# wenxuanliu/multimodal-vae

Hardware: AMD Instinct MI355X
Metric: ELBO-steps/sec (whole node), MultiMNIST b=256 per GPU (higher is better)
Workload: dtype bf16; 1 GPU; multimnist_50x50_conv_mmvae_gru_text_3pass_elbo_step; batch_per_gpu=256, global_batch=256, n_latents=100, parallelism=dp1, hip_graph=False, optimizer=adam, mfma=bf16 in / fp32 acc; fp32 master weights, BN stats, PoE/KL/BCE/NLL, Adam

## Files before the change

multimodal-vae_amd/csrc/elementwise.hip:

```cpp
#include "elementwise.h"
#include "bn_dev.h"
#include <math.h>

namespace {

constexpr int TPB = 256;

__device__ __forceinline__ float exp_unfused(float x) {
    const float c = 0x1.715476p+0f, cc = 0x1.4ae0bep-26f;
    float ph = x * c;
    asm volatile("" : "+v"(ph));
    float pl = fmaf(x, c, -ph);
    pl = fmaf(x, cc, pl);
    const float e = rintf(ph);
    float r = ldexpf(__builtin_amdgcn_exp2f((ph - e) + pl), (int)e);
    r = x < -0x1.9d1dap+6f ? 0.f : r;
    r = x > 0x1.62e43p+6f ? INFINITY : r;
    return r;
}
inline int nblocks(long long n, int per = TPB, int cap = 4096) {
    long long b = (n + per - 1) / per;
    if (b < 1) b = 1;
    if (b > cap) b = cap;
    return (int)b;
// ... 666 lines not shown
        a.z_bf[(size_t)b * a.ldz + a.D + c] = (bf16)(c == 0 ? 1.f : 0.f);
    }
    __shared__ double part[TPB / 64];
    kl = wave_sum_f64(kl);
    if ((threadIdx.x & 63) == 0) part[threadIdx.x >> 6] = kl;
    __syncthreads();
    if (threadIdx.x == 0) {
        double s = 0.0;
        for (int w = 0; w < TPB / 64; ++w) s += part[w];
        reinterpret_cast<double*>(a.scratch)[blockIdx.x] = s;
    }
}
__global__ void latent1_fwd_finish_kernel(const double* parts, float* kl_sum) {
    if (threadIdx.x != 0 || blockIdx.x != 0) return;
    double s = 0.0;
    for (int p = 0; p < LATENT1_KL_PARTS; ++p) s += parts[p];
    *kl_sum += (float)s;
}
__global__ __launch_bounds__(TPB) void latent1_bwd_kernel(const Latent1BwdArgs a) {
    const Latent1Args& f = a.f;
    const int D2 = 2 * f.D;
    const int tx = threadIdx.x & 63, ty = threadIdx.x >> 6;
    const int d = blockIdx.x * 64 + tx;
    __shared__ double red[2][4][64];
    double s_mu = 0.0, s_lv = 0.0;
    const int b_end = min(f.B, (int)(blockIdx.y + 1) * LATENT1_BWD_ROWS);
    for (int b = blockIdx.y * LATENT1_BWD_ROWS + ty; b < b_end; b += 4) {
        if (d < f.D) {
            const int e = b * f.D + d;
            double dz = a.dz ? (double)a.dz[e] : 0.0;
            if (a.dz2) dz += (double)a.dz2[e];
            const double mu = f.mu[e], lv = f.logvar[e], kc = a.kl_coef;
            const double gmu = dz + kc * mu;
            double glv = -0.5 * kc * (1.0 - exp(lv));
            if (f.training) glv += dz * (double)f.eps[e] * 0.5 * exp(0.5 * lv);
            a.d_enc_out[(size_t)b * a.ld + d] = (bf16)(float)gmu;
            a.d_enc_out[(size_t)b * a.ld + f.D + d] = (bf16)(float)glv;
            s_mu += gmu; s_lv += glv;
        }
        if (blockIdx.x == 0)
            for (int c = D2 + tx; c < a.ld; c += 64) a.d_enc_out[(size_t)b * a.ld + c] = (bf16)0.f;
    }
    if (!a.d_bias) return;
    red[0][ty][tx] = s_mu; red[1][ty][tx] = s_lv;
    __syncthreads();
    if (ty == 0 && d < f.D) {
        double* row = reinterpret_cast<double*>(f.scratch) + (size_t)blockIdx.y * D2;
        row[d] = red[0][0][tx] + red[0][1][tx] + red[0][2][tx] + red[0][3][tx];
        row[f.D + d] = red[1][0][tx] + red[1][1][tx] + red[1][2][tx] + red[1][3][tx];
    }
}
__global__ __launch_bounds__(TPB) void latent1_bwd_finish_kernel(const double* parts, int nrows, int D2, float* d_bias, const float* loss_slots,
                                                                 float* loss_out) {
    const int c = threadIdx.x;
    if (loss_slots && c < 16) {
        float t = 0.f;
        for (int q = 0; q < MMVAE_LOSS_SLOTS; ++q) t += loss_slots[q * 16 + c];
        loss_out[c] = t;
    }
    if (!d_bias || c >= D2) return;
    double s = 0.0;
    for (int r = 0; r < nrows; ++r) s += parts[(size_t)r * D2 + c];
    d_bias[c] += (float)s;
}
__global__ __launch_bounds__(TPB) void latent1_bwd_f32_kernel(const Latent1BwdF32Args a) {
    const long long n = (long long)a.B * a.ld;
    for (long long i = (long long)blockIdx.x * TPB + threadIdx.x; i < n; i += (long long)gridDim.x * TPB) {
        const int b = (int)(i / a.ld), c = (int)(i - (long long)b * a.ld);
        float v = 0.f;
        if (c < 2 * a.D) {
            const bool is_mu = c < a.D;
            const int e = b * a.D + (is_mu ? c : c - a.D);
            const double dz = a.dz ? (double)a.dz[e] : 0.0;
            const double mu = a.mu[e], lv = a.logvar[e], kc = a.kl_coef;
            const double gmu = dz + kc * mu;
            double glv = -0.5 * kc * (1.0 - exp(lv));
            if (a.training) glv += dz * (double)a.eps[e] * 0.5 * exp(0.5 * lv);
            v = is_mu ? (float)gmu : (float)glv;
        }
        a.d_enc_out[i] = v;
    }
}

__global__ __launch_bounds__(TPB) void adam_kernel(const AdamArgs a, unsigned* done) {
    const long long t = *a.step + 1;
    const bool skip = done[1] != 0u || (__float_as_uint(a.g[0]) & 0x7fffffffu) == MMVAE_VOID_MARK;
    const float bc1 = 1.0f - powf(a.b1, (float)t);
    const float bc2 = 1.0f - powf(a.b2, (float)t);
    const float step_size = a.lr / bc1;
    const float inv_sqrt_bc2 = rsqrtf(bc2);
    long long vbase[5];
    vbase[0] = 0;
#pragma unroll
    for (int r = 0; r < 4; ++r) vbase[r + 1] = vbase[r] + (r < a.nr ? (a.rlen[r] + 3) / 4 : 0);
    for (long long i = (long long)blockIdx.x * TPB + threadIdx.x; i < vbase[4] && !skip; i += (long long)gridDim.x * TPB) {
        int r = 0;
#pragma unroll
        for (int q = 1; q < 4; ++q) r += (q < a.nr && i >= vbase[q]) ? 1 : 0;
        const long long e = a.roff[r] + (i - vbase[r]) * 4, r_end = a.roff[r] + a.rlen[r];
        if (e + 4 <= r_end) {
            f32x4 g = *reinterpret_cast<const f32x4*>(a.g + e);
            if (a.gmap) {
                const int4 mi = *reinterpret_cast<const int4*>(a.gmap + e);
                const int mm[4] = {mi.x, mi.y, mi.z, mi.w};
#pragma unroll
                for (int j = 0; j < 4; ++j)
                    if (mm[j] >= 0) g[j] += a.gpk[mm[j]];
                    else if (mm[j] < -1) g[j] += a.gpk_vec[-mm[j] - 2];
                *reinterpret_cast<f32x4*>(a.g_out + e) = g;
            }
            f32x4 m = *reinterpret_cast<const f32x4*>(a.m + e);
            f32x4 v = *reinterpret_cast<const f32x4*>(a.v + e);
            f32x4 p = *reinterpret_cast<const f32x4*>(a.p + e);
#pragma unroll
            for (int j = 0; j < 4; ++j) {
                float gj = g[j] * a.grad_scale;
                m[j] = a.b1 * m[j] + (1.f - a.b1) * gj;
                v[j] = a.b2 * v[j] + (1.f - a.b2) * gj * gj;
                p[j] -= step_size * m[j] / (sqrtf(v[j]) * inv_sqrt_bc2 + a.eps);
            }
            *reinterpret_cast<f32x4*>(a.m + e) = m;
            *reinterpret_cast<f32x4*>(a.v + e) = v;
            *reinterpret_cast<f32x4*>(a.p + e) = p;
        } else {
            for (long long q = e; q < r_end; ++q) {
                float gq = a.g[q];
                if (a.gmap) {
                    const int mq = a.gmap[q];
                    if (mq >= 0) gq += a.gpk[mq]; else if (mq < -1) gq += a.gpk_vec[-mq - 2];
                    a.g_out[q] = gq;
                }
                float gj = gq * a.grad_scale;
                float m = a.b1 * a.m[q] + (1.f - a.b1) * gj;
                float v = a.b2 * a.v[q] + (1.f - a.b2) * gj * gj;
                a.m[q] = m; a.v[q] = v;
                a.p[q] -= step_size * m / (sqrtf(v) * inv_sqrt_bc2 + a.eps);
            }
        }
    }
    __syncthreads();
    if (threadIdx.x == 0) {
        unsigned ticket = atomicAdd(done, 1u);
        if (ticket == gridDim.x - 1) {
            done[0] = 0u;
            done[1] = 0u;
            if (!skip && !a.no_advance) *a.step = t;
            __threadfence();
        }
    }
}

__global__ __launch_bounds__(TPB) void embed_gather_stats_kernel(const float* table, int C, const long long* idx, int rows, int idx_rows,
                                                                 int rows_per_group, bf16* x, int ld, float2* colstats) {
    const int r0 = blockIdx.x * 64;
    for (int c = threadIdx.x & 63; c < ld; c += 64) {
        float s1 = 0.f, s2 = 0.f;
        int g_cur = -1;
        for (int rr = threadIdx.x >> 6; rr < 64; rr += TPB / 64) {
            const int r = r0 + rr;
            if (r >= rows) break;
            const int g = r / rows_per_group;
            if (g != g_cur && g_cur >= 0 && c < C && colstats) {
                atomicAdd(&colstats[(g_cur * MMVAE_STAT_SLOTS + blockIdx.x % MMVAE_STAT_SLOTS) * C + c].x, s1);
                atomicAdd(&colstats[(g_cur * MMVAE_STAT_SLOTS + blockIdx.x % MMVAE_STAT_SLOTS) * C + c].y, s2);
                s1 = s2 = 0.f;
            }
            g_cur = g;
            float v = 0.f;
            if (c < C) v = table[idx[r % idx_rows] * C + c];
            const bf16 b = (bf16)v;
            x[(size_t)r * ld + c] = b;
            const float vb = (float)b;
            s1 += vb; s2 += vb * vb;
        }
        if (g_cur >= 0 && c < C && colstats) {
            atomicAdd(&colstats[(g_cur * MMVAE_STAT_SLOTS + blockIdx.x % MMVAE_STAT_SLOTS) * C + c].x, s1);
            atomicAdd(&colstats[(g_cur * MMVAE_STAT_SLOTS + blockIdx.x % MMVAE_STAT_SLOTS) * C + c].y, s2);
        }
    }
}
__global__ __launch_bounds__(TPB) void embed_scatter_add_kernel(const bf16* d, int ld, int C, const long long* idx, int rows, float* g_table) {
    const int i = blockIdx.x * TPB + threadIdx.x;
    if (i >= rows * C) return;
    const int r = i / C, c = i - r * C;
    atomicAdd(g_table + idx[r] * C + c, (float)d[(size_t)r * ld + c]);
}
__global__ __launch_bounds__(TPB) void logsoftmax_nll_kernel(const LogSoftmaxNllArgs a) {
    const int r = blockIdx.x * TPB + threadIdx.x;
    float nll = 0.f;
    int g = 0;
    if (r < a.rows) {
        g = r / a.rows_per_group;
        const float* l = a.logits + (size_t)r * a.classes;
        float mx = -INFINITY;
        for (int c = 0; c < a.classes; ++c) mx = fmaxf(mx, l[c]);
        float se = 0.f;
        for (int c = 0; c < a.classes; ++c) se += exp_unfused(l[c] - mx);
        const float lg = logf(se);
        const int tg = a.target ? (int)a.target[r % a.target_rows] : -1;
        for (int c = 0; c < a.classes; ++c) {
            const float lp = (l[c] - mx) - lg;
            a.words[(size_t)r * a.classes + c] = lp;
            if (c == tg) nll = -lp;
            if (a.dlogits) a.dlogits[(size_t)r * a.ld_d + c] = (bf16)(a.coef[g & 3] * (exp_unfused(lp) - (c == tg ? 1.f : 0.f)));
            if (a.dlogits_f32) a.dlogits_f32[(size_t)r * a.classes + c] = a.coef[g & 3] * (exp_unfused(lp) - (c == tg ? 1.f : 0.f));
        }
        if (a.dlogits)
            for (int c = a.classes; c < a.ld_d; ++c) a.dlogits[(size_t)r * a.ld_d + c] = (bf16)0.f;
    }
    if (a.nll_sum && a.target) {
        if (a.rows_per_group % 64 == 0) {
            float s = wave_sum(nll);
            if ((threadIdx.x & 63) == 0 && r < a.rows) atomicAdd(a.nll_sum + (blockIdx.x % MMVAE_LOSS_SLOTS) * 16 + g, s);
        } else if (r < a.rows) {
            atomicAdd(a.nll_sum + (r % MMVAE_LOSS_SLOTS) * 16 + g, nll);
        }
    }
}
__global__ __launch_bounds__(TPB) void cast_bf16_kernel(const float* x, long long n, bf16* out) {
    const long long i = ((long long)blockIdx.x * TPB + threadIdx.x) * 4;
    if (i + 4 <= n) {
        const f32x4 v = *reinterpret_cast<const f32x4*>(x + i);
        bf16x4 o;
        for (int j = 0; j < 4; ++j) o[j] = (bf16)v[j];
        *reinterpret_cast<bf16x4*>(out + i) = o;
    } else {
        for (long long q = i; q < n; ++q) out[q] = (bf16)x[q];
    }
}
__global__ __launch_bounds__(TPB) void mse_fwd_kernel(const float* a, const float* b, long long n, float* out) {
    float acc = 0.f;
    for (long long i = (long long)blockIdx.x * TPB + threadIdx.x; i < n; i += (long long)gridDim.x * TPB) {
        const float d = a[i] - b[i];
        acc += d * d;
// ... 206 lines not shown
    MMVAE_REQUIRE(out != nullptr && n >= 0, "normal: null output or n=%lld < 0", n);
    if (n == 0) return MMVAE_OK;
    hipLaunchKernelGGL(normal_kernel, dim3(nblocks((n + 3) / 4, TPB, 512)), dim3(TPB), 0, s, out, n, seed, step, stream_id);
    return mmvae_check_launch("normal");
}
int launch_keep_mask(uint8_t* out, long long n, float p, unsigned long long seed, const long long* step, unsigned stream_id, hipStream_t s) {
    MMVAE_REQUIRE(out != nullptr && n >= 0, "keep_mask: null output or n=%lld < 0", n);
    MMVAE_REQUIRE(p >= 0.0f && p <= 1.0f, "keep_mask: p=%g is no probability in [0, 1]", (double)p);
    if (n == 0) return MMVAE_OK;
    hipLaunchKernelGGL(keep_mask_kernel, dim3(nblocks((n + 3) / 4, TPB, 512)), dim3(TPB), 0, s, out, n, p, seed, step, stream_id);
    return mmvae_check_launch("keep_mask");
}
int launch_latent3_fwd(const Latent3Args& a, hipStream_t s) {
    MMVAE_REQUIRE(a.B >= 1 && a.D >= 1 && a.ldz >= a.D && a.ldz % 8 == 0 && (long long)a.B * a.ldz <= 0x3FFFFFFF,
                  "latent3: B=%d D=%d ldz=%d", a.B, a.D, a.ldz);
    MMVAE_REQUIRE(a.img_out && a.txt_out && a.mu && a.logvar && a.z_f32 && a.z_bf && a.kl_sum && (!a.training || a.eps), "latent3: null argument");
    MMVAE_LAUNCH(latent3_fwd_kernel, dim3(nblocks((long long)a.B * a.ldz, TPB, 256)), dim3(TPB), 0, s, a);
    return mmvae_check_launch("latent3_fwd");
}
int launch_latent3_bwd(const Latent3BwdArgs& a, hipStream_t s) {
    MMVAE_REQUIRE((a.loss_slots == nullptr) == (a.loss_out == nullptr), "latent3_bwd: loss_slots / loss_out go together");
    MMVAE_REQUIRE(a.f.B >= 1 && a.f.D >= 1 && (long long)a.f.B * a.f.D <= 0x3FFFFFFF && ceil_div(a.f.B, L3B_ROWS) <= 65535,
                  "latent3_bwd: B=%d D=%d out of range", a.f.B, a.f.D);
    MMVAE_REQUIRE(a.f.img_out && a.f.txt_out && a.f.mu && a.f.logvar && (!a.f.training || a.f.eps), "latent3_bwd: null argument");
    MMVAE_REQUIRE(a.d_img_out_f32 || a.d_img_out_bf, "latent3_bwd: no image gradient output (d_img_out_f32 or d_img_out_bf)");
    MMVAE_REQUIRE(a.ld_img_out_bf == 0 || (a.ld_img_out_bf >= 2 * a.f.D && a.ld_img_out_bf % 8 == 0),
                  "latent3_bwd: ld_img_out_bf=%d is no multiple of 8 >= 2D", a.ld_img_out_bf);
    MMVAE_LAUNCH(latent3_bwd_kernel, dim3(ceil_div(a.f.D, 64), ceil_div(a.f.B, L3B_ROWS)), dim3(TPB), 0, s, a);
    return mmvae_check_launch("latent3_bwd");
}
size_t launch_latent1_scratch_floats(int B, int D) {
    const size_t fwd = 2 * (size_t)LATENT1_KL_PARTS, bwd = 2 * (size_t)ceil_div(B, LATENT1_BWD_ROWS) * 2 * D;
    return bwd > fwd ? bwd : fwd;
}
static int latent1_check(const Latent1Args& a, const char* who) {
    MMVAE_REQUIRE(a.B >= 1 && a.D >= 1 && a.D <= 128 && (long long)a.B * a.D <= 0x3FFFFFFF, "%s: B=%d D=%d out of range (D <= 128)", who, a.B, a.D);
    MMVAE_REQUIRE(a.mu && a.logvar && a.scratch && (!a.training || a.eps), "%s: null argument", who);
    MMVAE_REQUIRE(((uintptr_t)a.scratch & 7) == 0, "%s: scratch must be 8-byte aligned", who);
    return MMVAE_OK;
}
int launch_latent1_fwd(const Latent1Args& a, hipStream_t s) {
    MMVAE_TRY(latent1_check(a, "latent1_fwd"));
    MMVAE_REQUIRE(a.enc_out && a.z_f32 && a.z_bf && a.kl_sum, "latent1_fwd: null argument");
    MMVAE_REQUIRE(a.ldz >= a.D, "latent1_fwd: ldz=%d < D=%d", a.ldz, a.D);
    hipLaunchKernelGGL(latent1_fwd_kernel, dim3(LATENT1_KL_PARTS), dim3(TPB), 0, s, a);
    MMVAE_TRY(mmvae_check_launch("latent1_fwd"));
    MMVAE_LAUNCH(latent1_fwd_finish_kernel, dim3(1), dim3(64), 0, s, (const double*)a.scratch, a.kl_sum);
    return mmvae_check_launch("latent1_fwd_finish");
}
int launch_latent1_bwd(const Latent1BwdArgs& a, hipStream_t s) {
    MMVAE_TRY(latent1_check(a.f, "latent1_bwd"));
    MMVAE_REQUIRE(a.d_enc_out && a.ld >= 2 * a.f.D, "latent1_bwd: d_enc_out missing or ld=%d < 2D", a.ld);
    MMVAE_REQUIRE((a.loss_slots == nullptr) == (a.loss_out == nullptr), "latent1_bwd: loss_slots / loss_out go together");
    const int nrows = ceil_div(a.f.B, LATENT1_BWD_ROWS);
    hipLaunchKernelGGL(latent1_bwd_kernel, dim3(ceil_div(a.f.D, 64), nrows), dim3(TPB), 0, s, a);
    MMVAE_TRY(mmvae_check_launch("latent1_bwd"));
    if (!a.d_bias && !a.loss_slots) return MMVAE_OK;
    MMVAE_LAUNCH(latent1_bwd_finish_kernel, dim3(1), dim3(TPB), 0, s, (const double*)a.f.scratch, nrows, 2 * a.f.D, a.d_bias, a.loss_slots, a.loss_out);
    return mmvae_check_launch("latent1_bwd_finish");
}
int launch_latent1_bwd_f32(const Latent1BwdF32Args& a, hipStream_t s) {
    MMVAE_REQUIRE(a.B >= 1 && a.D >= 1 && a.D <= 128 && (long long)a.B * a.D <= 0x3FFFFFFF, "latent1_bwd_f32: B=%d D=%d out of range (D <= 128)", a.B, a.D);
    MMVAE_REQUIRE(a.mu && a.logvar && a.d_enc_out && (!a.training || a.eps), "latent1_bwd_f32: null argument");
    MMVAE_REQUIRE(a.ld >= 2 * a.D && (long long)a.B * a.ld <= 0x3FFFFFFF, "latent1_bwd_f32: ld=%d out of range (>= 2D)", a.ld);
    const int nb = ceil_div(a.B * a.ld, TPB);
    hipLaunchKernelGGL(latent1_bwd_f32_kernel, dim3(nb < 1024 ? nb : 1024), dim3(TPB), 0, s, a);
    return mmvae_check_launch("latent1_bwd_f32");
}
int launch_adam(const AdamArgs& a_in, hipStream_t s) {
    AdamArgs a = a_in;
    MMVAE_REQUIRE(a.step != nullptr, "adam: step counter is null");
    MMVAE_REQUIRE(a.p && a.g && a.m && a.v, "adam: null parameter, gradient or moment buffer");
    MMVAE_REQUIRE(a.n >= 1, "adam: n=%lld elements (the kernel reads g[0])", a.n);
    MMVAE_REQUIRE(a.gmap == nullptr || (a.gpk && a.gpk_vec && a.g_out), "adam: gradient map without packed gradient buffers");
    MMVAE_REQUIRE(a.nr >= 0 && a.nr <= 4, "adam: at most 4 element ranges");
    if (a.nr == 0) { a.nr = 1; a.roff[0] = 0; a.rlen[0] = a.n; }
    long long vecs = 0;
    for (int r = 0; r < a.nr; ++r) {
        MMVAE_REQUIRE(a.roff[r] >= 0 && a.rlen[r] >= 0 && a.roff[r] % 4 == 0 && a.roff[r] + a.rlen[r] <= a.n &&
                      (a.rlen[r] % 4 == 0 || a.roff[r] + a.rlen[r] == a.n), "adam: range %d = (%lld, %lld) of %lld elements", r, a.roff[r], a.rlen[r], a.n);
        vecs += (a.rlen[r] + 3) / 4;
    }
    unsigned* done = reinterpret_cast<unsigned*>(a.step + 1);
    hipLaunchKernelGGL(adam_kernel, dim3(nblocks(vecs > 0 ? vecs : 1, TPB, mmvae_knob(K_adam_blocks))), dim3(TPB), 0, s, a, done);
    return mmvae_check_launch("adam");
}
static __global__ __launch_bounds__(256) void gather_rows_kernel(const char* __restrict__ src, const long long* __restrict__ idx,
                                                                 long long row_bytes, int parts, char* __restrict__ dst) {
    const long long row = blockIdx.x / parts;
    const int part = blockIdx.x % parts;
    const long long vecs = row_bytes / 16, per = (vecs + parts - 1) / parts;
    const long long v0 = part * per, v1 = v0 + per < vecs ? v0 + per : vecs;
    const u32x4* s = reinterpret_cast<const u32x4*>(src + idx[row] * row_bytes);
    u32x4* d = reinterpret_cast<u32x4*>(dst + row * row_bytes);
    for (long long v = v0 + threadIdx.x; v < v1; v += 256) d[v] = s[v];
}
static __global__ __launch_bounds__(256) void gather_rows4_kernel(const char* __restrict__ src, const long long* __restrict__ idx,
                                                                  long long row_bytes, char* __restrict__ dst) {
    const long long row = blockIdx.x;
    const unsigned* s = reinterpret_cast<const unsigned*>(src + idx[row] * row_bytes);
    unsigned* d = reinterpret_cast<unsigned*>(dst + row * row_bytes);
    for (long long v = threadIdx.x; v < row_bytes / 4; v += 256) d[v] = s[v];
}
static __global__ __launch_bounds__(256) void gather_rows_u8_f32_kernel(const unsigned char* __restrict__ src, const long long* __restrict__ idx,
                                                                       long long row_elems, float denom, float* __restrict__ dst) {
    const long long row = blockIdx.x;
    const unsigned* s = reinterpret_cast<const unsigned*>(src + idx[row] * row_elems);
    f32x4* d = reinterpret_cast<f32x4*>(dst + row * row_elems);
    for (long long v = threadIdx.x; v < row_elems / 4; v += 256) {
        const unsigned w = s[v];
        d[v] = f32x4{(float)(w & 255u) / denom, (float)((w >> 8) & 255u) / denom, (float)((w >> 16) & 255u) / denom, (float)(w >> 24) / denom};
    }
}
int launch_gather_rows_u8_f32(const unsigned char* src, const long long* idx, long long rows, long long row_elems, float denom, float* dst, hipStream_t s) {
    MMVAE_REQUIRE(src && idx && dst && rows >= 1 && rows < (1ll << 31) && row_elems >= 4 && row_elems % 4 == 0 && ((uintptr_t)src & 3) == 0 &&
                  ((uintptr_t)dst & 15) == 0, "gather_rows_u8_f32: rows of a multiple of 4 elements, aligned buffers");
    hipLaunchKernelGGL(gather_rows_u8_f32_kernel, dim3((unsigned)rows), dim3(256), 0, s, src, idx, row_elems, denom, dst);
    return mmvae_check_launch("gather_rows_u8_f32");
}
int launch_gather_rows(const void* src, const long long* idx, long long rows, long long row_bytes, void* dst, hipStream_t s) {
    if (src && idx && dst && rows >= 1 && row_bytes >= 4 && row_bytes % 16 != 0) {
        MMVAE_REQUIRE(row_bytes % 4 == 0 && ((uintptr_t)src & 3) == 0 && ((uintptr_t)dst & 3) == 0 && rows < (1ll << 31), "gather_rows: rows of a multiple of 4 bytes, 4-byte aligned buffers");
        hipLaunchKernelGGL(gather_rows4_kernel, dim3((unsigned)rows), dim3(256), 0, s, (const char*)src, idx, row_bytes, (char*)dst);
        return mmvae_check_launch("gather_rows");
    }
    MMVAE_REQUIRE(src && idx && dst && rows >= 1 && row_bytes >= 16 && row_bytes % 16 == 0, "gather_rows: rows of a multiple of 16 bytes");
    MMVAE_REQUIRE(((uintptr_t)src & 15) == 0 && ((uintptr_t)dst & 15) == 0, "gather_rows: 16-byte aligned buffers");
    int parts = (int)((row_bytes + 32767) / 32768);
    if (parts < 1) parts = 1;
    MMVAE_REQUIRE(rows * parts < (1ll << 31), "gather_rows: too many rows");
    hipLaunchKernelGGL(gather_rows_kernel, dim3((unsigned)(rows * parts)), dim3(256), 0, s, (const char*)src, idx, row_bytes, parts, (char*)dst);
    return mmvae_check_launch("gather_rows");
}
static __global__ void step_losses_kernel(StepLossArgs a) {
    const int k = threadIdx.x;
    if (k < 3) a.out[k] = a.w_bce[k] * a.sums[k] + a.w_nll[k] * a.sums[4 + k] + a.w_kl[k] * a.sums[8 + k];
}
int launch_step_losses(const StepLossArgs& a, hipStream_t s) {
    MMVAE_REQUIRE(a.sums && a.out, "step_losses: null buffer");
    hipLaunchKernelGGL(step_losses_kernel, dim3(1), dim3(64), 0, s, a);
    return mmvae_check_launch("step_losses");
}
int launch_fill_zero(void* p, size_t bytes, hipStream_t s) {
    if (hipMemsetAsync(p, 0, bytes, s) != hipSuccess) {
        mmvae_set_error("hipMemsetAsync failed");
        return MMVAE_EHIP;
    }
    return MMVAE_OK;
}

int launch_bce_fwd(const float* p, const float* t, long long n, float* out, hipStream_t s) {
    hipLaunchKernelGGL(bce_fwd_kernel, dim3(nblocks(n, TPB * 4, 1024)), dim3(TPB), 0, s, p, t, n, out);
    return mmvae_check_launch("bce_fwd");
}
int launch_bce_bwd(const float* p, const float* t, long long n, float coef, const float* gs, float* dp, hipStream_t s) {
    hipLaunchKernelGGL(bce_bwd_kernel, dim3((unsigned)((n + TPB - 1) / TPB)), dim3(TPB), 0, s, p, t, n, coef, gs, dp);
    return mmvae_check_launch("bce_bwd");
}
int launch_nll_fwd(const float* lp, const long long* tg, int rows, int classes, float* out, hipStream_t s) {
    hipLaunchKernelGGL(nll_fwd_kernel, dim3(nblocks(rows, TPB, 64)), dim3(TPB), 0, s, lp, tg, rows, classes, out);
    return mmvae_check_launch("nll_fwd");
}
int launch_nll_bwd(const long long* tg, int rows, int classes, float coef, const float* gs, float* dlp, hipStream_t s) {
    hipLaunchKernelGGL(nll_bwd_kernel, dim3(ceil_div(rows * classes, TPB)), dim3(TPB), 0, s, tg, rows, classes, coef, gs, dlp);
    return mmvae_check_launch("nll_bwd");
}

// ... 85 lines not shown
```

multimodal-vae_amd/csrc/knobs.h:

```cpp
#pragma once
#include <atomic>

#define MMVAE_KNOBS(KNOB) \
    KNOB(convres, 1, AB, "image-resident conv kernels (convres.hip); 0: every layer on gemm_gather, except launches with a staging transform, which exist only there") \
    KNOB(convres_celeba, 1, AB, "convres.hip on the 64x64 image tower's layers (CelebA, COCO); 0: those layers on gemm_gather") \
    KNOB(convres_alt, 0, AB, "convres.hip tile configurations: 1 hallucinate.6 with 4 images per workgroup, 3 no direct-B kernels, 4 no split bottleneck kernels, 5 no 16-image hallucinate.0") \
    KNOB(convres_dbg, 0, MEASURE, "convres kernels leave phases out (bit mask, tools/convres_check.py)") \
    KNOB(convres_ts_lo, 0, ADDR, "convres kernels: time stamps of workgroup 0's phases, low half of the pointer") \
    KNOB(convres_ts_hi, 0, ADDR, "high half") \
    KNOB(mm_fuse_bn, 1, AB, "MultiMNIST step: BatchNorm passes folded into the staging of the image-resident conv kernels; 0: the unfused bn_act + gather-GEMM chain") \
    KNOB(ca_fuse_bn, 1, AB, "the same for the 64x64 image tower (CelebA, COCO)") \
    KNOB(mm_stage_out, 1, AB, "the staging conv kernels leave the activated operand / BatchNorm-backward dr behind for the weight gradient; 0: materialised on the side stream in front of it") \
    KNOB(mm_conv1_mfma, 1, AB, "MultiMNIST features.0 forward and weight gradient on conv1.hip; 0: gemm_gather") \
    KNOB(dec_last_mfma, 1, AB, "MultiMNIST decoder tail (hallucinate.9 + BCE + its gradients) on dec_last.hip; 0: separate launches") \
    KNOB(dec_last_ca, 1, AB, "the 64x64 tower's decoder tail on dec_last.hip; 0: separate launches") \
    KNOB(dec_last_ca_dbg, 0, MEASURE, "64x64 decoder tail leaves work out: bit 0 logits, 1 patches, 2 input gradient, 3 weight gradient, 4 P") \
    KNOB(wgrad_ring, 1, AB, "ring-staged weight-gradient kernels (wgrad_ring.hip); 0: the streamed gemm_gather form") \
    KNOB(wr_pair, 0, AB, "1: the two-classes-per-workgroup geometries of wgrad_ring.hip (tried and lost, DESIGN)") \
    KNOB(wr_wgs, -1, TUNE, "workgroups of a ring launch in quarters of the CU count; -1: 4 from 4e9 MACs, else 3") \
    KNOB(wr_wgs_big, 0, TUNE, "the same for a geometry that names its own (G::WGQ); 0: the geometry's") \
    KNOB(wr_bias, 6, TUNE, "fixed cost of a batch for a ring workgroup, in column tiles, when image groups are dealt to classes") \
    KNOB(wr_run, 0, TUNE, "consecutive jobs dealt to one XCD residue by the ring launch's workgroup order; 0: one per job class and channel slice") \
    KNOB(wr_xcd, 1, AB, "0: ring jobs in sorted order, not dealt to the XCDs") \
    KNOB(wr_atomic_kb, 256, TUNE, "a ring launch adds into the packed gradient by fp32 atomics up to this many KB of dW; above: partial copies + reduce") \
    KNOB(wr_dbg, 0, MEASURE, "ring kernels leave phases out (bit mask, tools/wgrad_check.py)") \
    KNOB(wr_ts_lo, 0, ADDR, "ring kernels: time stamps of workgroup 0's phases, low half of the pointer") \
    KNOB(wr_ts_hi, 0, ADDR, "high half") \
    KNOB(wgrad_atomic, 0, AB, "1: streamed weight gradients add into the packed gradient by fp32 atomics, no slab / reduce") \
    KNOB(batch_reduce, 1, AB, "one reduce launch per flushed side stream; 0: one behind every weight gradient") \
    KNOB(mm_wgrad_inline, 0, AB, "1: MultiMNIST image weight gradients on the main stream (no fork, no join); 2: and their partial copies summed by one launch in front of the optimizer") \
    KNOB(one_wgrad_stream, 0, AB, "1: one weight-gradient side stream instead of two") \
    KNOB(side_lanes, 3, AB, "bit 0: lane-1 side work goes to the second-modality stream; bit 1: lane 2 to the spare weight-gradient stream") \
    KNOB(mm_cls_lane, 1, AB, "side-stream lane of the classifier's grouped weight gradients") \
    KNOB(mm_conv3_lane, 0, AB, "side-stream lane of features.5's weight gradient") \
    KNOB(mm_conv4_lane, 0, AB, "side-stream lane of features.8's weight gradient") \
    KNOB(mm_forks, 0, AB, "1: one fork for the whole encoder / decoder backward instead of one per flush point") \
    KNOB(one_join, -1, AB, "end of step: 1 the side streams meet on one of them and the main stream waits once, 0 it waits for each; -1: once when there are two weight-gradient streams") \
    KNOB(ev_flags, 2, AB, "flags of the step's events: 2 no system-scope fence, 0 HIP's default fence (read when an event is created)") \
    KNOB(no_stop_events, 0, AB, "1: forks are event records on the main stream, not the producer kernel's completion signal") \
    KNOB(adam_blocks, 512, TUNE, "workgroup cap of the Adam kernel") \
    KNOB(begin_blocks, 2048, TUNE, "zero / random-number workgroup cap of the step prologue") \
    KNOB(mm_dz_event, 1, AB, "the main chain joins the text decoder backward on that kernel's own event; 0: on everything enqueued on its stream") \
    KNOB(mm_stage_begin, 1, AB, "staged prologue: the main stream refreshes only what the image encoder's forward reads, the rest on the second-modality stream; 0: one launch") \
    KNOB(mm_early_adam, 1, AB, "the decoders' Adam update runs beside the encoders' backward when the caller passes early_adam; 0: never") \
    KNOB(mm_image_waist, -1, AB, "image-only MultiMNIST step: 1 / 0 the one-expert waist kernels on / off where compiled; -1: the size's default (1 at n_latents = 20, 0 at 100)") \
    KNOB(mnist_strip, -1, AB, "image-only MNIST step: 1 / 0 the column-strip Linear + BatchNorm kernels on / off up to 512 rows; -1: the default, 1") \
    KNOB(text_fwd2, 1, AB, "MultiMNIST text decoder forward: the weights-resident text_decoder_fwd2_kernel at the reference's sizes; 0: the streamed form at every size") \
    KNOB(txt_ts_lo, 0, ADDR, "text decoder forward: time stamps of workgroup 0's phases, low half of the pointer") \
    KNOB(txt_ts_hi, 0, ADDR, "high half") \
    KNOB(pack_runs, 1, AB, "every weight pack: the lanes of a wave walk the source's contiguous direction (pack_geo.h); 0: the row-major assignment it replaced, reference of tests/test_gpu_pack_runs.py") \
    KNOB(pack_stage_grid, 1, AB, "a staged prologue launch holds only its own descriptors' workgroups and the zero / random workgroups it needs; 0: the whole table and begin_blocks workgroups in every launch") \
    KNOB(gemm_small_prefetch, 2, AB, "gemm_small_kernel with 2 .. 4 64-deep chunks of both operands in flight per wave; 0: gemm_small_kernel_v0, reference of tests/test_gpu_gemm_small_forms.py") \
    KNOB(dbg_skip_wgrad, 0, MEASURE, "the step without weight gradients: 1 all, 2 ring-staged, 3 streamed, 4 grouped") \
    KNOB(dbg_skip_text, 0, MEASURE, "1: the step without its text kernels") \
    KNOB(dbg_skip_edges, 0, MEASURE, "the step without event edges: 1 all, 2 forks (main -> side), 3 joins") \
    KNOB(dbg_begin_skip, 0, MEASURE, "prologue without: bit 0 the pack, 1 the random draws, 2 the workspace zeroing") \
    KNOB(dbg_begin_skip_zero, 0, MEASURE, "prologue without zeroing: bit 0 the packed gradient, 1 the gradients") \
    KNOB(dbg_text_rows_div, 0, MEASURE, "n > 0: the text decoder on 1/n of its rows") \
    KNOB(coco_cluster, 8, AB, "ranks per 16-row block of the caption decoder's persistent launches: 8, 4, or 0 / 1 one workgroup per block") \
    KNOB(coco_enc_streamed, 0, AB, "1: the caption encoder's weight-streaming kernels instead of the weight-resident ones") \
    KNOB(coco_no_comb, 0, AB, "1: the cluster-of-8 decoder's three-exchange kernels instead of the composed two-exchange form") \
    KNOB(coco_no_comb_bwd, 0, AB, "1: the composed form off in the decoder's backward only") \
    KNOB(coco_no_mse_fuse, 0, AB, "1: the caption MSE not fused into the composed decoder forward") \
    KNOB(coco_module_bf16, 0, AB, "caption module entry points: 0 the fp32 kernels; 1 the step's bf16 persistent kernels on the module's B rows; 2 their forward without saving, backward refuses") \
    KNOB(celeba_layer_mask, 0, AB, "mmvae_celeba_bench_layer: 1 the dropout keep flags take part in the fc layers") \
    KNOB(coco_layer_mask, 0, AB, "mmvae_coco_bench_layer: 1 the dropout keep flags in m1 / m2 take part in the fc layers")

enum MmvaeKnob {
#define KNOB(name, dflt, kind, doc) K_##name,
    MMVAE_KNOBS(KNOB)
#undef KNOB
    K_COUNT
};

extern std::atomic<int> g_mmvae_knobs[K_COUNT];
static inline int mmvae_knob(MmvaeKnob k) { return g_mmvae_knobs[k].load(std::memory_order_relaxed); }
static inline unsigned long long* mmvae_knob_ptr(MmvaeKnob lo, MmvaeKnob hi) {
    return reinterpret_cast<unsigned long long*>(((unsigned long long)(unsigned)mmvae_knob(hi) << 32) | (unsigned)mmvae_knob(lo));
}
```

multimodal-vae_amd/csrc/multimnist.hip:

```cpp
#include "multimnist.h"
#include <memory>
#include "mlp_tail.h"
#include "plan_base.h"
#include "thin.h"
#include "text_plan.h"
#include <cstring>

namespace {
constexpr int IMG = 50, NPIX = 2500;
}

struct MMPlan : PlanBase {
    int ldz, kx, kz;
    int lde;
    ConvL conv[4], convT[4];
    LinL fc[3], up;
    BnL bn[6];
    int H = TXT_H;
    const char *te_name = "text_encoder", *td_name = "text_decoder";
    TextGruIdx te_f, te_r, td0, td1;
    const float* step_image = nullptr;
    hipEvent_t ev_dz = nullptr;
    hipEvent_t ev_txtgrads = nullptr;
    int te_h2p, te_h2pT, g_te_h2p, td_z2h, td_z2hT, g_td_z2h, td_h2o, td_h2oT, g_td_h2o;
// ... 700 lines not shown
TextDecArgs td_args(MMPlan& P, const float* z, int groups, bool save) { return text_dec_args(P, z, groups, save); }
int txt_dec_bwd(MMPlan& P, const TextDecArgs& f, const float* dwords, float* dz, hipStream_t s) {
    const int R = f.R;
    const TextDecBwdArgs a = text_dec_bwd_args(P, f, dwords, dz);
    P.ev_dz = nullptr;
    const bool own_ev = P.in_step && s == P.st_text && mmvae_knob(K_mm_dz_event) != 0;
    if (own_ev) {
        P.ev_dz = next_ev(P);
        if (!P.capturing && !mmvae_knob(K_no_stop_events)) mmvae_arm_stop_event(P.ev_dz);
    }
    MMVAE_TRY(launch_text_decoder_bwd(a, s));
    if (own_ev && (mmvae_take_stop_event() != nullptr || P.capturing || mmvae_knob(K_no_stop_events)) && hipEventRecord(P.ev_dz, s) != hipSuccess) {
        mmvae_set_error("text decoder event failed: %s", hipGetErrorString(hipGetLastError()));
        return MMVAE_EHIP;
    }
    MMVAE_TRY(text_dec_wgrads(P, R, s));
    P.ev_txtgrads = nullptr;
    if (own_ev) {
        P.ev_txtgrads = next_ev(P);
        if (hipEventRecord(P.ev_txtgrads, s) != hipSuccess) {
            mmvae_set_error("text decoder event failed: %s", hipGetErrorString(hipGetLastError()));
            return MMVAE_EHIP;
        }
    }
    return MMVAE_OK;
}

}

MMPlan* mm_create(int D, int B) {
    if (D < 1 || D > 127 || B < 1) { mmvae_set_error("mm_create: need 1 <= n_latents <= 127 and batch >= 1"); return nullptr; }
    MMPlan* P = new MMPlan();
    P->D = D; P->B = B;
    P->single_wgrad_stream = true;
    build_plan(*P);
    plan_size_workspaces(*P, carve);
    return P;
}
void mm_destroy(MMPlan* P) { delete P; }
int mm_early_ranges(const MMPlan* P, long long* ranges, int cap) {
    int n = 0;
    for (const ParamInfo& pi : P->params) {
        if (pi.name.rfind("image_decoder.", 0) != 0 && pi.name.rfind("text_decoder.", 0) != 0) continue;
        if (n > 0 && ranges[2 * (n - 1)] + ranges[2 * (n - 1) + 1] == pi.offset) { ranges[2 * (n - 1) + 1] += pi.numel; continue; }
        if (n == cap) return 0;
        ranges[2 * n] = pi.offset; ranges[2 * n + 1] = pi.numel; ++n;
    }
    for (int r = 0; r < n; ++r)
        if (ranges[2 * r] % 4 != 0 || ranges[2 * r + 1] % 4 != 0) return 0;
    return n;
}
PlanBase* mm_base(MMPlan* P) { return P; }

static int use_ws(MMPlan* P, void* ws, size_t bytes, bool module = true) { return plan_use_ws(P, ws, bytes, module, carve); }

static int mm_step_body(MMPlan* Pp, const mmvae_mm_step_io& io, int training, int do_backward, hipStream_t s);
int mm_step_fwd_bwd(MMPlan* Pp, const mmvae_mm_step_io& io, int training, int do_backward, hipStream_t s) {
    if (const mmvae_early_adam* e = io.early_adam) {
        MMVAE_REQUIRE(e->m && e->v && e->state && e->gmap && e->ran, "mmvae_mm_step: early_adam with a null field");
        *e->ran = 0;
    }
    return plan_step(Pp, io, training, do_backward, s, mm_step_body);
}
static int mm_step_body(MMPlan* Pp, const mmvae_mm_step_io& io, int training, int do_backward, hipStream_t s) {
    MMVAE_TRY(use_ws(Pp, io.ws, io.ws_bytes, false));
    MMPlan& P = *Pp;
    MMPlan::W& w = P.w;
    const int B = P.B, D = P.D, B3 = 3 * B;
    MMVAE_REQUIRE(io.image && io.text && io.sums, "step: image/text/sums must be given");
    const float* eps = io.eps;
    const uint8_t *m1 = io.enc_mask1, *m2 = io.enc_mask2, *gk = io.gru_keep;
    const bool serial0 = mmvae_serial();
    const bool staged = mmvae_knob(K_mm_stage_begin) != 0 && !serial0;
    StepBeginArgs sb{}, sb2{};
    sb.zero_ptr[0] = w.zero_begin; sb.zero_bytes[0] = w.zero_bytes;
    StepBeginArgs& sz = staged ? sb2 : sb;
    if (do_backward) {
        sz.zero_ptr[1] = P.buf.gpk; sz.zero_bytes[1] = (size_t)P.gk.mat_elems * sizeof(float);
        sz.zero_ptr[2] = P.buf.grads; sz.zero_bytes[2] = (size_t)(P.nparams / 4) * 16;
        const int skipz = mmvae_knob(K_dbg_begin_skip_zero);
        if (skipz & 1) sz.zero_ptr[1] = nullptr;
        if (skipz & 2) sz.zero_ptr[2] = nullptr;
    }
    sb.p = DROP_P; sb.seed = io.seed; sb.step = io.step_counter;
    if (training && !eps) { sb.eps = w.eps; sb.n_eps = (long long)B3 * D; eps = w.eps; }
    if (training && io.enc_dropout && !m1) { sb.mask[0] = w.m1; sb.n_mask[0] = (long long)2 * B * 400; m1 = w.m1; }
    if (training && io.enc_dropout && !m2) { sb.mask[1] = w.m2; sb.n_mask[1] = (long long)2 * B * 200; m2 = w.m2; }
    if (training && io.gru_dropout && !gk) { sb.mask[2] = w.gkeep; sb.n_mask[2] = (long long)4 * B3 * P.H; gk = w.gkeep; }
    const int skipb = mmvae_knob(K_dbg_begin_skip);
    if (skipb & 2) { sb.eps = nullptr; sb.mask[0] = sb.mask[1] = sb.mask[2] = nullptr; }
    if (skipb & 4) sb.zero_ptr[0] = nullptr;
    const bool pack_now = io.pack_first && !(skipb & 1);
    if (pack_now) {
        MMVAE_TRY(step_begin_with_pack(sb, P.buf.desc_dev, P.pk.d.data(), (int)P.pk.d.size(), P.buf.params, P.buf.packed, P.buf.packed_vec,
                                       staged ? 1u << 0 : 0u));
    }
    MMVAE_TRY(ensure_streams(P));
    P.in_step = true;
    {
        hipStreamCaptureStatus cs = hipStreamCaptureStatusNone;
        P.capturing = hipStreamIsCapturing(s, &cs) == hipSuccess && cs == hipStreamCaptureStatusActive;
    }
    arm_fork(P);
    MMVAE_TRY(launch_step_begin(sb, s));
    MMVAE_TRY(commit_fork(P, s));
    if (do_backward && P.nparams % 4 != 0)
        MMVAE_TRY(launch_fill_zero(P.buf.grads + (P.nparams / 4) * 4, (size_t)(P.nparams % 4) * sizeof(float), s));
    const int enc_drop = training && io.enc_dropout;
    const int sk[3] = {io.pass_skip[0] != 0, io.pass_skip[1] != 0, io.pass_skip[2] != 0};
    P.dec_skip_mask = (unsigned)(sk[0] | (sk[1] << 1) | (sk[2] << 2));
    const int enc_updates = 2 - sk[0] - sk[1];
    const bool serial = mmvae_serial();
    hipStream_t T = serial ? s : P.st_text;
    if (T != s) MMVAE_TRY(fork_to(P, T));
    if (staged && pack_now) {
        StepBeginArgs st1{};
        MMVAE_TRY(step_begin_with_pack(st1, P.buf.desc_dev, P.pk.d.data(), (int)P.pk.d.size(), P.buf.params, P.buf.packed, P.buf.packed_vec, 1u << 1));
        MMVAE_TRY(launch_step_begin(st1, T));
    }
    {
        TextEncArgs a = te_args(P, io.text, w.txtout, do_backward);
        MMVAE_TRY(launch_text_encoder_fwd(a, T));
    }
    if (staged && (pack_now || sb2.zero_ptr[1] || sb2.zero_ptr[2])) {
        if (pack_now)
            MMVAE_TRY(step_begin_with_pack(sb2, P.buf.desc_dev, P.pk.d.data(), (int)P.pk.d.size(), P.buf.params, P.buf.packed, P.buf.packed_vec, 1u << 2));
        MMVAE_TRY(launch_step_begin(sb2, T));
    }
    P.step_image = io.image;
    const bool fuse = mmvae_knob(K_mm_fuse_bn) != 0 && mmvae_knob(K_convres) != 0 && B % 8 == 0;
    MMVAE_TRY(enc_fwd(P, io.image, 2, m1, m2, enc_drop, training, enc_updates, w.encout, s, fuse));
    MMVAE_TRY(edge(P, T, s));
    Latent3Args la{};
    la.B = B; la.D = D; la.img_out = w.encout; la.txt_out = w.txtout; la.eps = eps;
    la.mu = io.mu ? io.mu : w.mu; la.logvar = io.logvar ? io.logvar : w.logvar;
    la.z_f32 = w.z_f32; la.z_bf = w.z_bf; la.ldz = P.ldz; la.kl_sum = w.sums + 8; la.training = training;
    arm_fork(P);
    MMVAE_TRY(launch_latent3_fwd(la, s));
    MMVAE_TRY(commit_fork(P, s));
    if (T != s) MMVAE_TRY(fork_to(P, T));
    TextDecArgs td = td_args(P, w.z_f32, 3, do_backward);
    td.keep = (training && io.gru_dropout) ? gk : nullptr; td.keep_scale = 1.f / (1.f - DROP_P);
    td.force_tokens = io.force_tokens;
    if (io.recon_text) td.words = io.recon_text;
    if (io.tokens) td.tokens_out = io.tokens;
    td.target = io.text; td.nll_sum = w.sums + 4; td.dwords = do_backward ? w.dwords : nullptr;
    for (int k = 0; k < 3; ++k) td.nll_coef[k] = sk[k] ? 0.f : io.lambda_yx[k] / (float)(B * TXT_T);
    if (const int half = mmvae_knob(K_dbg_text_rows_div)) td.R = max(16, td.R / half);
    MMVAE_TRY(launch_text_decoder_fwd(td, T));
    if (do_backward) MMVAE_TRY(txt_dec_bwd(P, td, w.dwords, w.dz_txt, T));
    ConvTLastFwdArgs last{};
    last.target = io.image; last.recon = io.recon_image; last.dlogit = do_backward ? w.dlogit : nullptr; last.loss_sum = w.sums;
    for (int k = 0; k < 3; ++k) last.coef[k] = sk[k] ? 0.f : io.lambda_xy[k] / (float)(B * NPIX);
    int last_groups = 3;
    if (!io.recon_image)
        while (last_groups > 1 && last.coef[last_groups - 1] == 0.f) --last_groups;
    int img_groups = 3;
    while (img_groups > 0 && (io.lambda_xy[img_groups - 1] == 0.f || sk[img_groups - 1])) --img_groups;
    const bool fuse_tail = P.slab.pool != nullptr;
    MMVAE_TRY(dec_fwd(P, 3, training, &last, s, last_groups, fuse_tail ? (do_backward ? std::min(img_groups, last_groups) : 0) : -1, fuse));
    if (!do_backward) {
        MMVAE_TRY(edge(P, T, s));
        P.in_step = false;
        hipLaunchKernelGGL(sum_slots_kernel, dim3(1), dim3(64), 0, s, w.sums, io.sums);
        return mmvae_check_launch("sum_slots");
    }

    P.wgrad_forked = mmvae_knob(K_mm_wgrad_inline) == 0;
    int rc = MMVAE_OK;
    P.deferred.clear();
    P.defer_wgrad = false;
    if (img_groups > 0) rc = dec_bwd(P, w.dlogit, img_groups, w.dz_img, s, fuse_tail, fuse, 3, training);
    if (io.early_adam && rc == MMVAE_OK && img_groups > 0 && fuse && fuse_tail && P.wgrad_forked && !serial && T != s && !io.dp_split &&
        io.defer_unpack && P.ev_txtgrads && P.side_pending.empty() && P.st_wgrad2 == P.st_wgrad && mmvae_knob(K_mm_early_adam)) {
        hipStream_t Wst = P.st_wgrad;
        AdamArgs ad{};
        const mmvae_early_adam& ea = *io.early_adam;
        ad.p = P.buf.params; ad.g = P.buf.grads; ad.m = ea.m; ad.v = ea.v; ad.n = P.nparams; ad.step = ea.state;
        ad.lr = ea.lr; ad.b1 = ea.beta1; ad.b2 = ea.beta2; ad.eps = ea.eps; ad.grad_scale = ea.grad_scale;
        ad.gmap = ea.gmap; ad.gpk = P.buf.gpk; ad.gpk_vec = P.buf.gpk_vec; ad.g_out = P.buf.grads;
        long long rg[8];
        ad.nr = mm_early_ranges(&P, rg, 4);
        for (int r = 0; r < ad.nr; ++r) { ad.roff[r] = rg[2 * r]; ad.rlen[r] = rg[2 * r + 1]; }
        ad.no_advance = 1;
        if (ad.nr > 0) {
            if (hipStreamWaitEvent(Wst, P.ev_txtgrads, 0) != hipSuccess) { mmvae_set_error("early optimizer part: %s", hipGetErrorString(hipGetLastError())); rc = MMVAE_EHIP; }
            if (rc == MMVAE_OK) rc = launch_adam(ad, Wst);
            if (rc == MMVAE_OK) *ea.ran = 1;
        }
    }
    if (rc == MMVAE_OK) {
        const int k = mmvae_knob(K_dbg_skip_edges);
        if (P.ev_dz && T != s) {
            if (k != 1 && k != 3 && hipStreamWaitEvent(s, P.ev_dz, 0) != hipSuccess) {
                mmvae_set_error("stream join failed: %s", hipGetErrorString(hipGetLastError()));
                rc = MMVAE_EHIP;
            }
        } else {
            rc = edge(P, T, s);
        }
// ... 444 lines not shown
```

Before: 1838 ELBO-steps/s.

## Add software-pipelined Adam kernel and move latent/GRU draws to the text stream

Adds a templated Adam kernel that keeps two or three 4-element vectors in flight per thread, issuing gradient-map gathers together to hide memory latency. It is selected by a new knob that defaults to the old kernel. The staged MultiMNIST prologue now draws eps and the GRU keep flags in the text stream's stage-1 launch instead of the main stream's stage 0. This shortens the work that precedes the image encoder on the main stream. The risk is extra launch work on the text stream, which could delay the text encoder.

```diff
diff --git a/multimodal-vae_amd/csrc/elementwise.hip b/multimodal-vae_amd/csrc/elementwise.hip
--- a/multimodal-vae_amd/csrc/elementwise.hip
+++ b/multimodal-vae_amd/csrc/elementwise.hip
@@ -772,7 +772,7 @@
     }
 }
 
-__global__ __launch_bounds__(TPB) void adam_kernel(const AdamArgs a, unsigned* done) {
+__global__ __launch_bounds__(TPB) void adam_kernel_v0(const AdamArgs a, unsigned* done) {
     const long long t = *a.step + 1;
     const bool skip = done[1] != 0u || (__float_as_uint(a.g[0]) & 0x7fffffffu) == MMVAE_VOID_MARK;
     const float bc1 = 1.0f - powf(a.b1, (float)t);
@@ -840,6 +840,145 @@
     }
 }
 
+struct AdamSlot {
+    long long e;
+    bool whole;
+    int4 mi;
+    f32x4 g, m, v, p;
+    float x[4];
+};
+__device__ __forceinline__ void adam_locate(const AdamArgs& a, const long long (&vbase)[5], long long i, long long safe_e, AdamSlot& s) {
+    long long off = a.roff[0], len = a.rlen[0], base = 0;
+#pragma unroll
+    for (int q = 1; q < 4; ++q)
+        if (q < a.nr && i >= vbase[q]) { off = a.roff[q]; len = a.rlen[q]; base = vbase[q]; }
+    const long long e = off + (i - base) * 4;
+    s.whole = i < vbase[4] && e + 4 <= off + len;
+    s.e = s.whole ? e : safe_e;
+}
+template <bool MAP> __device__ __forceinline__ void adam_load_map(const AdamArgs& a, AdamSlot& s) {
+    if (MAP) s.mi = *reinterpret_cast<const int4*>(a.gmap + s.e);
+}
+__device__ __forceinline__ void adam_load_operands(const AdamArgs& a, AdamSlot& s) {
+    s.g = *reinterpret_cast<const f32x4*>(a.g + s.e);
+    s.m = *reinterpret_cast<const f32x4*>(a.m + s.e);
+    s.v = *reinterpret_cast<const f32x4*>(a.v + s.e);
+    s.p = *reinterpret_cast<const f32x4*>(a.p + s.e);
+}
+template <bool FUSED_V>
+__device__ __forceinline__ void adam_element(const AdamArgs& a, float step_size, float inv_sqrt_bc2, float g, float& m, float& v, float& p) {
+    const float gj = g * a.grad_scale;
+    m = fmaf(a.b1, m, (1.f - a.b1) * gj);
+    float q = (1.f - a.b2) * gj * gj;
+    if (FUSED_V) {
+        v = fmaf(a.b2, v, q);
+    } else {
+        float bv = a.b2 * v;
+        asm volatile("" : "+v"(bv));
+        asm volatile("" : "+v"(q));
+        v = bv + q;
+    }
+    p = p - step_size * m / fmaf(sqrtf(v), inv_sqrt_bc2, a.eps);
+}
+template <bool MAP> __device__ __forceinline__ void adam_gather(const AdamArgs& a, AdamSlot& s) {
+    if (!MAP) return;
+    const int mm[4] = {s.mi.x, s.mi.y, s.mi.z, s.mi.w};
+#pragma unroll
+    for (int j = 0; j < 4; ++j) {
+        const float* src = mm[j] >= 0 ? a.gpk + mm[j] : mm[j] < -1 ? a.gpk_vec + (-mm[j] - 2) : a.g + s.e + j;
+        s.x[j] = *src;
+    }
+}
+template <bool MAP> __device__ __forceinline__ void adam_apply(const AdamArgs& a, const AdamSlot& s, float step_size, float inv_sqrt_bc2) {
+    const long long e = s.e;
+    f32x4 g = s.g, m = s.m, v = s.v, p = s.p;
+    if (MAP) {
+        const int mm[4] = {s.mi.x, s.mi.y, s.mi.z, s.mi.w};
+#pragma unroll
+        for (int j = 0; j < 4; ++j)
+            if (mm[j] != -1) g[j] += s.x[j];
+    }
+#pragma unroll
+    for (int j = 0; j < 4; ++j) {
+        float mj = m[j], vj = v[j], pj = p[j];
+        adam_element<true>(a, step_size, inv_sqrt_bc2, g[j], mj, vj, pj);
+        m[j] = mj; v[j] = vj; p[j] = pj;
+    }
+    if (s.whole) {
+        if (MAP) *reinterpret_cast<f32x4*>(a.g_out + e) = g;
+        *reinterpret_cast<f32x4*>(a.m + e) = m;
+        *reinterpret_cast<f32x4*>(a.v + e) = v;
+        *reinterpret_cast<f32x4*>(a.p + e) = p;
+    }
+}
+__device__ __forceinline__ void adam_tail(const AdamArgs& a, long long e, long long r_end, float step_size, float inv_sqrt_bc2) {
+    for (long long q = e; q < r_end; ++q) {
+        float gq = a.g[q];
+        if (a.gmap) {
+            const int mq = a.gmap[q];
+            if (mq >= 0) gq += a.gpk[mq]; else if (mq < -1) gq += a.gpk_vec[-mq - 2];
+            a.g_out[q] = gq;
+        }
+        float m = a.m[q], v = a.v[q], p = a.p[q];
+        adam_element<false>(a, step_size, inv_sqrt_bc2, gq, m, v, p);
+        a.m[q] = m; a.v[q] = v; a.p[q] = p;
+    }
+}
+template <int DEPTH, bool MAP>
+__global__ __launch_bounds__(TPB) void adam_kernel(const AdamArgs a, unsigned* done) {
+    const long long t = *a.step + 1;
+    const bool skip = done[1] != 0u || (__float_as_uint(a.g[0]) & 0x7fffffffu) == MMVAE_VOID_MARK;
+    if (!skip) {
+        long long vbase[5];
+        vbase[0] = 0;
+#pragma unroll
+        for (int r = 0; r < 4; ++r) vbase[r + 1] = vbase[r] + (r < a.nr ? (a.rlen[r] + 3) / 4 : 0);
+        long long safe_e = -1;
+#pragma unroll
+        for (int r = 3; r >= 0; --r)
+            if (r < a.nr && a.rlen[r] >= 4) safe_e = a.roff[r];
+        const long long stride = (long long)gridDim.x * TPB;
+        long long wg = (long long)blockIdx.x * TPB, i = wg + threadIdx.x;
+        const float bc1 = 1.0f - powf(a.b1, (float)t);
+        const float bc2 = 1.0f - powf(a.b2, (float)t);
+        const float step_size = a.lr / bc1;
+        const float inv_sqrt_bc2 = rsqrtf(bc2);
+        if (safe_e >= 0 && wg < vbase[4]) {
+            AdamSlot s[DEPTH + 1];
+#pragma unroll
+            for (int k = 0; k < DEPTH; ++k) { adam_locate(a, vbase, i + k * stride, safe_e, s[k]); adam_load_map<MAP>(a, s[k]); }
+#pragma unroll
+            for (int k = 0; k + 1 < DEPTH; ++k) { adam_load_operands(a, s[k]); adam_gather<MAP>(a, s[k]); }
+            for (bool more = true; more;) {
+#pragma unroll
+                for (int u = 0; u <= DEPTH; ++u) {
+                    if (wg >= vbase[4]) { more = false; break; }
+                    adam_load_operands(a, s[(u + DEPTH - 1) % (DEPTH + 1)]);
+                    adam_gather<MAP>(a, s[(u + DEPTH - 1) % (DEPTH + 1)]);
+                    adam_locate(a, vbase, i + DEPTH * stride, safe_e, s[(u + DEPTH) % (DEPTH + 1)]);
+                    adam_load_map<MAP>(a, s[(u + DEPTH) % (DEPTH + 1)]);
+                    adam_apply<MAP>(a, s[u], step_size, inv_sqrt_bc2);
+                    i += stride; wg += stride;
+                }
+            }
+        }
+#pragma unroll
+        for (int r = 0; r < 4; ++r)
+            if (r < a.nr && (a.rlen[r] & 3) != 0 && (vbase[r + 1] - 1) % stride == (long long)blockIdx.x * TPB + threadIdx.x)
+                adam_tail(a, a.roff[r] + (a.rlen[r] & ~3ll), a.roff[r] + a.rlen[r], step_size, inv_sqrt_bc2);
+    }
+    __syncthreads();
+    if (threadIdx.x == 0) {
+        unsigned ticket = atomicAdd(done, 1u);
+        if (ticket == gridDim.x - 1) {
+            done[0] = 0u;
+            done[1] = 0u;
+            if (!skip && !a.no_advance) *a.step = t;
+            __threadfence();
+        }
+    }
+}
+
 __global__ __launch_bounds__(TPB) void embed_gather_stats_kernel(const float* table, int C, const long long* idx, int rows, int idx_rows,
                                                                  int rows_per_group, bf16* x, int ld, float2* colstats) {
     const int r0 = blockIdx.x * 64;
@@ -1212,7 +1351,14 @@
         vecs += (a.rlen[r] + 3) / 4;
     }
     unsigned* done = reinterpret_cast<unsigned*>(a.step + 1);
-    hipLaunchKernelGGL(adam_kernel, dim3(nblocks(vecs > 0 ? vecs : 1, TPB, mmvae_knob(K_adam_blocks))), dim3(TPB), 0, s, a, done);
+    const dim3 grid(nblocks(vecs > 0 ? vecs : 1, TPB, mmvae_knob(K_adam_blocks)));
+    const int depth = mmvae_knob(K_adam_pipeline);
+    MMVAE_REQUIRE(depth == 0 || depth == 2 || depth == 3, "adam: knob adam_pipeline = %d (0, 2 or 3)", depth);
+    if (depth == 0) hipLaunchKernelGGL(adam_kernel_v0, grid, dim3(TPB), 0, s, a, done);
+    else if (depth == 2 && a.gmap) hipLaunchKernelGGL((adam_kernel<2, true>), grid, dim3(TPB), 0, s, a, done);
+    else if (depth == 2) hipLaunchKernelGGL((adam_kernel<2, false>), grid, dim3(TPB), 0, s, a, done);
+    else if (a.gmap) hipLaunchKernelGGL((adam_kernel<3, true>), grid, dim3(TPB), 0, s, a, done);
+    else hipLaunchKernelGGL((adam_kernel<3, false>), grid, dim3(TPB), 0, s, a, done);
     return mmvae_check_launch("adam");
 }
 static __global__ __launch_bounds__(256) void gather_rows_kernel(const char* __restrict__ src, const long long* __restrict__ idx,
diff --git a/multimodal-vae_amd/csrc/knobs.h b/multimodal-vae_amd/csrc/knobs.h
--- a/multimodal-vae_amd/csrc/knobs.h
+++ b/multimodal-vae_amd/csrc/knobs.h
@@ -39,6 +39,8 @@
     KNOB(ev_flags, 2, AB, "flags of the step's events: 2 no system-scope fence, 0 HIP's default fence (read when an event is created)") \
     KNOB(no_stop_events, 0, AB, "1: forks are event records on the main stream, not the producer kernel's completion signal") \
     KNOB(adam_blocks, 512, TUNE, "workgroup cap of the Adam kernel") \
+    KNOB(adam_pipeline, 0, AB, "2, 3: adam_kernel with that many 4-element vectors in flight per thread, gathers issued together (same bits, tests/test_gpu_adam_pipelined.py); 0: adam_kernel_v0, the default until the pipelined form's kernel time is measured (DESIGN 6)") \
+    KNOB(mm_stage_draws, 1, AB, "staged MultiMNIST prologue: eps and the text decoder's keep flags are drawn by the second-modality stream's stage-1 launch; 0: by the main stream's stage 0") \
     KNOB(begin_blocks, 2048, TUNE, "zero / random-number workgroup cap of the step prologue") \
     KNOB(mm_dz_event, 1, AB, "the main chain joins the text decoder backward on that kernel's own event; 0: on everything enqueued on its stream") \
     KNOB(mm_stage_begin, 1, AB, "staged prologue: the main stream refreshes only what the image encoder's forward reads, the rest on the second-modality stream; 0: one launch") \
diff --git a/multimodal-vae_amd/csrc/multimnist.hip b/multimodal-vae_amd/csrc/multimnist.hip
--- a/multimodal-vae_amd/csrc/multimnist.hip
+++ b/multimodal-vae_amd/csrc/multimnist.hip
@@ -806,13 +806,15 @@
         if (skipz & 1) sz.zero_ptr[1] = nullptr;
         if (skipz & 2) sz.zero_ptr[2] = nullptr;
     }
-    sb.p = DROP_P; sb.seed = io.seed; sb.step = io.step_counter;
-    if (training && !eps) { sb.eps = w.eps; sb.n_eps = (long long)B3 * D; eps = w.eps; }
+    StepBeginArgs st1{};
+    StepBeginArgs& sd = staged && mmvae_knob(K_mm_stage_draws) != 0 ? st1 : sb;
+    sb.p = st1.p = DROP_P; sb.seed = st1.seed = io.seed; sb.step = st1.step = io.step_counter;
+    if (training && !eps) { sd.eps = w.eps; sd.n_eps = (long long)B3 * D; eps = w.eps; }
     if (training && io.enc_dropout && !m1) { sb.mask[0] = w.m1; sb.n_mask[0] = (long long)2 * B * 400; m1 = w.m1; }
     if (training && io.enc_dropout && !m2) { sb.mask[1] = w.m2; sb.n_mask[1] = (long long)2 * B * 200; m2 = w.m2; }
-    if (training && io.gru_dropout && !gk) { sb.mask[2] = w.gkeep; sb.n_mask[2] = (long long)4 * B3 * P.H; gk = w.gkeep; }
+    if (training && io.gru_dropout && !gk) { sd.mask[2] = w.gkeep; sd.n_mask[2] = (long long)4 * B3 * P.H; gk = w.gkeep; }
     const int skipb = mmvae_knob(K_dbg_begin_skip);
-    if (skipb & 2) { sb.eps = nullptr; sb.mask[0] = sb.mask[1] = sb.mask[2] = nullptr; }
+    if (skipb & 2) { sb.eps = st1.eps = nullptr; sb.mask[0] = sb.mask[1] = sb.mask[2] = st1.mask[2] = nullptr; }
     if (skipb & 4) sb.zero_ptr[0] = nullptr;
     const bool pack_now = io.pack_first && !(skipb & 1);
     if (pack_now) {
@@ -837,9 +839,9 @@
     const bool serial = mmvae_serial();
     hipStream_t T = serial ? s : P.st_text;
     if (T != s) MMVAE_TRY(fork_to(P, T));
-    if (staged && pack_now) {
-        StepBeginArgs st1{};
-        MMVAE_TRY(step_begin_with_pack(st1, P.buf.desc_dev, P.pk.d.data(), (int)P.pk.d.size(), P.buf.params, P.buf.packed, P.buf.packed_vec, 1u << 1));
+    if (staged && (pack_now || st1.eps || st1.mask[2])) {
+        if (pack_now)
+            MMVAE_TRY(step_begin_with_pack(st1, P.buf.desc_dev, P.pk.d.data(), (int)P.pk.d.size(), P.buf.params, P.buf.packed, P.buf.packed_vec, 1u << 1));
         MMVAE_TRY(launch_step_begin(st1, T));
     }
     {
```

Result: no change. 1829 ELBO-steps/s (-0.5%).
